# sangho-vision/acav100m

Measured on AMD Instinct MI355X. Metric: clips/sec curated (k-means train + assign, 2 views) + MI greedy selection of 20 %, higher is better.
Workload: dtype f32

## Files before the change

acav100m_amd/_lib.py:

```python
import ctypes as C
import os

_HERE = os.path.dirname(os.path.abspath(__file__))
LIB_PATH = os.environ.get("ACAV_LIB_PATH") or os.path.join(_HERE, "libacav_hip.so")

vp, i64, i32, f32, f64, u32 = C.c_void_p, C.c_int64, C.c_int, C.c_float, C.c_double, C.c_uint32
pp = C.POINTER(C.c_void_p)

SIGNATURES = {
    "acav_version": [],
    "acav_device_count": [C.POINTER(i32)],
    "acav_device_info": [i32, C.c_char_p, i32, C.POINTER(i32), C.POINTER(i64)],
    "acav_trim_device_cache": [C.POINTER(i64)],
    "acav_rng_create": [pp, u32],
    "acav_rng_destroy": [vp],
    "acav_rng_seed": [vp, u32],
    "acav_rng_u32": [vp, C.POINTER(u32)],
    "acav_rng_jump": [vp, i64],
    "acav_rng_py_shuffle": [vp, i64, vp],
    "acav_rng_rand_f32": [vp, vp, i64],
    "acav_rng_randperm": [vp, i64, vp],
    "acav_rng_get_state": [vp, vp, C.POINTER(i32)],
    "acav_rng_set_state": [vp, vp, i32],
    "acav_rng_warmup_best": [vp, i32, i64, vp, C.POINTER(f32)],
    "acav_kmeans_create": [pp, i32, i32, i32, vp, vp],
    "acav_kmeans_destroy": [vp],
    "acav_kmeans_get_state": [vp, vp, vp, C.POINTER(i64), C.POINTER(i64)],
    "acav_kmeans_set_state": [vp, vp, vp, i64, i64],
    "acav_kmeans_set_hyper": [vp, i32, f64, f64],
    "acav_kmeans_assign": [vp, vp, i64, vp, C.POINTER(f32)],
    "acav_kmeans_step": [vp, vp, i64, f64, vp, C.POINTER(f32)],
    "acav_kmeans_train": [vp, vp, i64, i64, f64, vp, i64],
    "acav_kmeans_train_multi": [vp, i32, vp, vp, i64, f64, vp, vp],
    "acav_kmeans_train_form": [i32, i32, i64, i32, i32, i32, i32, i32, i32, i32, C.POINTER(i32)],
    "acav_kmeans_assign_plan": [i32, i32, i64, i32, i32, i32, i32, C.POINTER(i32)],
    "acav_kmeans_apply_update": [vp, vp, i64, vp, f64],
    "acav_kmeans_sync": [vp],
    "acav_kmeans_shape": [vp, C.POINTER(i32), C.POINTER(i32)],
    "acav_kmeans_stream": [vp, pp],
    "acav_comm_unique_id": [vp],
    "acav_comm_init": [pp, i32, i32, i32, vp, vp],
    "acav_comm_destroy": [vp],
    "acav_comm_info": [vp, C.POINTER(i32), C.POINTER(i32)],
    "acav_comm_sync": [vp],
    "acav_comm_allreduce_f32": [vp, vp, i64],
    "acav_comm_allgather": [vp, vp, vp, i64],
    "acav_comm_broadcast": [vp, vp, i64, i32],
    "acav_kmeans_allreduce_init": [vp, vp],
    "acav_kmeans_train_dp": [vp, vp, vp, i64, i64, f64, vp, i64, i64, i32],
    "acav_kmeans_train_dp_multi": [vp, vp, i32, vp, i64, i64, f64, vp, vp, i64, vp],
    "acav_kmeans_train_plan_multi": [vp, vp, i32, vp, i64, i32, i64, vp, i64, i64, f64, vp, vp, i64, vp],
    "acav_kmeans_broadcast_state": [vp, vp, i32],
    "acav_kmeans_timer_begin": [vp],
    "acav_kmeans_timer_end": [vp, C.POINTER(f32)],
    "acav_kmeans_stats": [vp, C.POINTER(i64), C.POINTER(i64)],
    "acav_kmeans_train_stats": [vp, C.POINTER(i64), C.POINTER(i64)],
    "acav_kmeans_filter_stats": [vp, C.POINTER(i64), C.POINTER(i64), C.POINTER(i64)],
    "acav_kmeans_recheck_stats": [vp, C.POINTER(i64), C.POINTER(i64), C.POINTER(i64)],
    "acav_kmeans_filter_time": [vp, C.POINTER(f32)],
    "acav_contrastive_create": [pp, i32, i32, i32, i32, vp, vp],
    "acav_contrastive_destroy": [vp],
    "acav_contrastive_get_params": [vp, vp, C.POINTER(i64)],
    "acav_contrastive_set_params": [vp, vp],
    "acav_contrastive_train": [vp, vp, vp, vp, i64, f64, vp, vp],
    "acav_contrastive_infer": [vp, vp, vp, i64, vp],
    "acav_contrastive_set_comm": [vp, vp],
    "acav_contrastive_backward": [vp, vp, vp, i64, vp, vp],
    "acav_contrastive_get_grads": [vp, vp],
    "acav_contrastive_set_grads": [vp, vp],
    "acav_contrastive_step": [vp, f64],
    "acav_mi_create": [pp, i32, vp, i64, i32, i32, vp, i32, vp],
    "acav_mi_destroy": [vp],
    "acav_mi_add_samples": [vp, vp, i64],
    "acav_mi_score_batch": [vp, vp, i32, vp],
    "acav_mi_run_greedy": [vp, vp, i64, vp, i32, i64, i32, i32, i32, vp, vp, vp, C.POINTER(i64),
                           C.POINTER(i64), vp, vp, vp, vp, i64],
    "acav_mi_run_greedy_multi": [vp, i32, vp, vp, vp, vp, vp, i32, i32, i32, vp, vp, vp, vp, vp],
    "acav_fy_block_grid": [i32, i32, i32, C.POINTER(i64)],
    "acav_fy_block_map": [i64, i32, i32, i32, C.POINTER(i32), C.POINTER(i32), C.POINTER(i32)],
    "acav_mi_run_exact": [vp, vp, i64, i32, i64, vp, vp, C.POINTER(i64), vp, vp, vp],
    "acav_mi_run_exact_multi": [vp, i32, vp, vp, vp, vp, vp, vp, vp],
    "acav_mi_run_celf": [vp, vp, i64, i32, i64, f64, vp, vp, vp, C.POINTER(i64), i64, vp, vp, vp],
    "acav_mi_set_measure": [vp, i32],
    "acav_mi_set_average_method": [vp, i32],
    "acav_mi_set_pair_weights": [vp, vp, i32],
    "acav_mi_get_pair_stats": [vp, vp, vp, vp, vp],
    "acav_mi_get_counts": [vp, vp, vp, vp, C.POINTER(i64)],
    "acav_mi_sync": [vp],
    "acav_mi_timer_begin": [vp],
    "acav_mi_timer_end": [vp, C.POINTER(f32)],
    "acav_pkl_shard_open": [C.c_char_p, pp],
    "acav_pkl_shard_close": [vp],
    "acav_pkl_shard_info": [vp, C.POINTER(i64), C.POINTER(i32), C.POINTER(i32)],
    "acav_pkl_shard_view": [vp, i32, C.POINTER(i32), C.POINTER(C.c_char_p), C.POINTER(C.c_char_p), C.POINTER(C.c_char_p),
                            C.POINTER(C.c_char_p), C.POINTER(i64)],
    "acav_pkl_shard_copy_view": [vp, i32, vp, i64],
    "acav_pkl_shard_meta": [vp, pp, C.POINTER(i64), pp, C.POINTER(i64), pp, pp, pp],
    "acav_pkl_load_group": [vp, i32, vp, vp, i32, vp, vp, vp, vp, vp, i32, vp, vp],
    "acav_pkl_assign_load_group": [vp, i32, i32, vp, vp],
    "acav_pkl_shard_labels": [vp, pp],
}

_lib = None
_FIRST_DEVICE_CALLS = ("acav_device_count", "acav_device_info", "acav_kmeans_create", "acav_mi_create",
                       "acav_contrastive_create", "acav_comm_init")
_device_touched = False


def device_touched():
    return _device_touched


def _marking(fn):
    def call(*args):
        global _device_touched
        _device_touched = True
        return fn(*args)
    call.argtypes, call.restype, call.__name__ = fn.argtypes, fn.restype, fn.__name__
    return call


class AcavError(RuntimeError):
    pass


def load_library():
    global _lib
    if _lib is not None:
        return _lib
    if not os.path.exists(LIB_PATH):
        raise AcavError(
            f"{LIB_PATH} is missing: run `python __graft_entry__.py` (hipcc --offload-arch=gfx950) first. "
            "There is no CPU fallback.")
    try:
        import torch
    except Exception:
        pass
    lib = C.CDLL(LIB_PATH)
    lib.acav_last_error.restype = C.c_char_p
    lib.acav_last_error.argtypes = []
    for name, args in SIGNATURES.items():
        fn = getattr(lib, name)
        fn.restype = i32
        fn.argtypes = args
    for name in _FIRST_DEVICE_CALLS:
        setattr(lib, name, _marking(getattr(lib, name)))
    _lib = lib
    return lib


def check(rc):
    if rc != 0:
        msg = _lib.acav_last_error().decode("utf-8", "replace") if _lib is not None else ""
        if rc == -1:
            raise ValueError(f"acav: {msg}")
        if rc == -5:
            raise RuntimeError(f"acav: {msg}")
        if rc == -7:
            raise TimeoutError(f"acav: {msg}")
        raise AcavError(f"acav error {rc}: {msg}")


def device_count():
    n = i32(0)
    check(load_library().acav_device_count(C.byref(n)))
    return n.value


def ptr(obj):
    if obj is None:
        return None
    if hasattr(obj, "data_ptr"):
        return C.c_void_p(obj.data_ptr())
    return obj.ctypes.data_as(C.c_void_p)
```

acav100m_amd/csrc/acav_common.h:

```cpp
#pragma once
#include <hip/hip_runtime.h>

#include <cstdarg>
#include <cstdint>
#include <cstdio>
#include <cstring>
#include <new>
#include <vector>

#include "../../include/acav_hip.h"

#define ACAV_EXPORT extern "C" __attribute__((visibility("default")))

#if (defined(ACAV_ABL_NOAFRAG) || defined(ACAV_ABL_NOCDMA) || defined(ACAV_ABL_NOMFMA) || defined(ACAV_ABL_NOXDMA) || \
     defined(ACAV_ABL_NOXDMA_G123) || defined(ACAV_ABL_XHALF_G123) || \
     defined(ACAV_DBG_HALF_CAND_WINDOW) || defined(ACAV_FY_ABL_BKSEQ) || defined(ACAV_FY_ABL_NOWALK) || defined(ACAV_FY_ABL_SRCSEQ) || defined(ACAV_MI_ABL_EMPTY)) && \
    !defined(ACAV_EXPERIMENT_BUILD)
#error "ACAV_ABL_* / ACAV_FY_ABL_* / ACAV_MI_ABL_* select timing-only kernels with wrong results: experiment harnesses only (-DACAV_EXPERIMENT_BUILD)"
#endif

namespace acav {

void set_error(const char *fmt, ...);

#define ACAV_HIP_TRY(expr)                                                                         \
    do {                                                                                           \
        hipError_t _e = (expr);                                                                    \
        if (_e != hipSuccess) {                                                                    \
            acav::set_error("%s failed: %s (%s:%d)", #expr, hipGetErrorString(_e), __FILE__, __LINE__); \
            return ACAV_EHIP;                                                                      \
        }                                                                                          \
    } while (0)

#define ACAV_REQUIRE(cond, code, ...)      \
    do {                                   \
        if (!(cond)) {                     \
            acav::set_error(__VA_ARGS__);  \
            return (code);                 \
        }                                  \
    } while (0)

#define ACAV_TRY(expr)             \
    do {                           \
        int _rc = (expr);          \
        if (_rc != ACAV_OK) return _rc; \
    } while (0)

bool is_device_ptr(const void *p);

void retire_stream(hipStream_t s);
void retire_event(hipEvent_t e);
void flush_retired(bool force);
int devbuf_alloc(void **p, size_t *bytes, size_t want, int *dev = nullptr);
void devbuf_free(void *p, size_t bytes, int dev = -1);
size_t devbuf_trim();

struct DevBuf {
    void *p = nullptr;
    size_t bytes = 0;
    int dev = -1;
    hipStream_t owner = nullptr;
    bool bound = false;
    ~DevBuf() { release(); }
    void bind(hipStream_t s) { owner = s, bound = true; }
    void release()
    {
        if (p) devbuf_free(p, bytes, dev);
        p = nullptr;
        bytes = 0;
    }
    int ensure(size_t n)
    {
        if (n <= bytes) return ACAV_OK;
        if (p) (void)(bound ? hipStreamSynchronize(owner) : hipDeviceSynchronize());
        release();
        return devbuf_alloc(&p, &bytes, n, &dev);
    }
    template <class T> T *as() const { return static_cast<T *>(p); }
};

int to_device(const void *src, size_t bytes, DevBuf &stage, hipStream_t stream, const void **out);
int upload(DevBuf &dst, const void *src, size_t bytes, hipStream_t stream);
int from_device(void *dst, const void *src_dev, size_t bytes, hipStream_t stream);

const uint32_t *mt_jump_poly(int64_t J);
int mt_jump_window_host(uint32_t *window, int64_t J);

struct StreamCtx {
    int device = 0;
    hipStream_t stream = nullptr;
    bool own_stream = false;
    hipEvent_t ev0 = nullptr, ev1 = nullptr;
    int init(int dev, void *user_stream, int priority_class = 0);
    void fini(bool retire = false);
    int timer_begin();
    int timer_end(float *ms);
};

}
```

acav100m_amd/csrc/acav_mi.hip:

```cpp
#include <algorithm>
#include <chrono>
#include <cmath>
#include <type_traits>

#include "acav_common.h"
#include <rocprim/rocprim.hpp>
#include <vector>

using namespace acav;

#ifdef ACAV_MI_ABL_EMPTY
#define ACAV_MI_EMPTY_RETURN return;
#else
#define ACAV_MI_EMPTY_RETURN
#endif

namespace {

struct MiScalars {
    long long nc;
};

#ifdef ACAV_FY_PROF
__device__ unsigned long long fy_prof[16];
// ... 1159 lines not shown
    const bool before = r > 0 && celf_val_geq(pm[r - 1], qval[order[r]]);
    if (here && !before) dn->kstop = r + 1;
}
__global__ __launch_bounds__(256) void k_celf_dense_winner(int n, const double *__restrict__ d, const double *__restrict__ pm,
                                                           CelfDense *__restrict__ dn)
{
    const int r = blockIdx.x * 256 + threadIdx.x;
    const int k = dn->kstop;
    if (r >= k) return;
    const double best = pm[k - 1], v = d[r];
    if ((v != v && best != best) || v == best) atomicMax(&dn->winner, r);
}
__global__ __launch_bounds__(256) void k_celf_dense_apply(int n, const int *__restrict__ A, const int *__restrict__ order,
                                                          const double *__restrict__ d, const CelfDense *__restrict__ dn,
                                                          const CelfState *__restrict__ state, double *__restrict__ qval,
                                                          long long *__restrict__ qst, long long *__restrict__ tr_ids,
                                                          double *__restrict__ tr_vals, int tr_cap)
{
    const int r = blockIdx.x * 256 + threadIdx.x;
    if (r >= dn->kstop) return;
    const int w = order[r];
    qval[w] = d[r];
    qst[w] = state->t + r + 1;
    if (r < tr_cap) {
        if (tr_ids) tr_ids[r] = (long long)A[w];
        if (tr_vals) tr_vals[r] = d[r];
    }
}
template <bool PAIR>
__global__ __launch_bounds__(256) void k_celf_dense_commit(CelfCtx c, const int *__restrict__ A, const int *__restrict__ order,
                                                           const double *__restrict__ d, const CelfDense *__restrict__ dn,
                                                           CelfState *state, unsigned char *removed,
                                                           long long *__restrict__ S_out, double *__restrict__ G_out,
                                                           long long *__restrict__ LK_out, long long *__restrict__ tr_ids,
                                                           double *__restrict__ tr_vals, int tr_cap)
{
    const int tid = threadIdx.x;
    const int k = dn->kstop, a = dn->winner;
    const int pos = order[a];
    const long long nc = c.sc->nc;
    const double gain0 = state->gain;
    const long long t0 = state->t;
    __syncthreads();
    if (tid == 0) {
        long long lk = k;
        if (a != k - 1) {
            if (k < tr_cap) {
                if (tr_ids) tr_ids[k] = (long long)A[pos];
                if (tr_vals) tr_vals[k] = d[a];
            }
            ++lk;
        }
        removed[pos] = 1;
        state->gain = gain0 + d[a];
        state->t = t0 + lk;
        *S_out = (long long)A[pos];
        *G_out = gain0 + d[a];
        *LK_out = lk;
        c.sc->nc = nc + 1;
    }
    celf_commit_tables<PAIR>(c, A[pos], tid);
}

__global__ void k_celf_queue_out(int L, const unsigned char *__restrict__ removed, const double *__restrict__ qval,
                                 double *__restrict__ out)
{
    const int w = blockIdx.x * blockDim.x + threadIdx.x;
    if (w < L) out[w] = removed[w] ? -INFINITY : qval[w];
}

__device__ __forceinline__ unsigned mt_temper(unsigned y)
{
    y ^= y >> 11;
    y ^= (y << 7) & 0x9d2c5680u;
    y ^= (y << 15) & 0xefc60000u;
    y ^= y >> 18;
    return y;
}
__device__ __forceinline__ unsigned mt_twist(unsigned y) { return (y >> 1) ^ ((y & 1u) ? 0x9908b0dfu : 0u); }

constexpr int MT_THREADS = 640;
constexpr int MT_WIDE = 623;
constexpr int MT_BACK = 1078;
constexpr int MT_EPOCH = 24;
constexpr int MT_WIN = MT_BACK + MT_WIDE * MT_EPOCH;
__device__ __forceinline__ void mt_generate_body(const unsigned *__restrict__ mt_state, unsigned *__restrict__ out, long long n)
{
    __shared__ unsigned X[MT_WIN];
    const unsigned tid = threadIdx.x;
    if (n <= 0) return;
    const long long p = (long long)mt_state[624];
    for (unsigned k = tid; k < 624; k += MT_THREADS) X[k] = mt_state[k];
    const long long q = p + n;
    const long long need = 624 * ((q - 1) / 624) + 624;
    __syncthreads();
    for (long long m = p + tid; m < 624 && m < q; m += MT_THREADS) out[m - p] = X[m];
    unsigned *outp = out + (624 - p);
    long long m0 = 624;
    long long shift = 0;
    for (; m0 < need && m0 < MT_BACK; m0 += 227) {
        if (tid < 227) {
            const unsigned w = (unsigned)m0 + tid;
            const unsigned v = X[w - 227] ^ mt_twist((X[w - 624] & 0x80000000u) | (X[w - 623] & 0x7fffffffu));
            X[w] = v;
            if ((long long)w < q) outp[w - 624] = v;
        }
        asm volatile("s_waitcnt lgkmcnt(0)" ::: "memory");
        __builtin_amdgcn_s_barrier();
    }
    const unsigned *xw = X + ((unsigned)(m0 - shift) + tid - MT_BACK);
    unsigned ob = ((unsigned)(m0 - p) + tid) * 4u;
    const unsigned ob_end = (unsigned)n * 4u;
    const char *outb = reinterpret_cast<const char *>(out);
    int left = MT_EPOCH;
    while (m0 < need) {
        if (left == 0) {
            unsigned keep[2];
            const unsigned src = (unsigned)(m0 - shift) - MT_BACK;
#pragma unroll
            for (int u = 0; u < 2; ++u) keep[u] = tid + u * MT_THREADS < MT_BACK ? X[src + tid + u * MT_THREADS] : 0u;
#pragma unroll
            for (int u = 0; u < 2; ++u)
                if (tid + u * MT_THREADS < MT_BACK) X[tid + u * MT_THREADS] = keep[u];
            __syncthreads();
            shift = m0 - MT_BACK;
            xw = X + tid;
            left = MT_EPOCH;
        }
        if (tid < MT_WIDE) {
            const unsigned a = xw[0] ^ xw[227] ^ xw[454], b2 = xw[1] ^ xw[228] ^ xw[455];
            const unsigned v = xw[MT_BACK - 681] ^ mt_twist((a & 0x80000000u) | (b2 & 0x7fffffffu));
            const_cast<unsigned *>(xw)[MT_BACK] = v;
            if (ob < ob_end) *reinterpret_cast<unsigned *>(const_cast<char *>(outb) + ob) = v;
        }
        xw += MT_WIDE;
        ob += MT_WIDE * 4u;
        m0 += MT_WIDE;
        --left;
        asm volatile("s_waitcnt lgkmcnt(0)" ::: "memory");
        __builtin_amdgcn_s_barrier();
    }
    __syncthreads();
}

__global__ __launch_bounds__(MT_THREADS) void k_mt_generate_lanes(unsigned *__restrict__ states, unsigned *__restrict__ out0,
                                                                 long long blk, long long head)
{
    ACAV_MI_EMPTY_RETURN
    const long long lane = blockIdx.x;
    const long long extra = lane == 0 ? head : 0;
    mt_generate_body(states + lane * 625, out0 + lane * blk - extra, blk + extra);
}

constexpr int MJ_WORDS = MT_BACK + MT_WIDE * 32;
__global__ __launch_bounds__(MT_THREADS) void k_mt_jump(unsigned *__restrict__ states, int src0, int dst0,
                                                       const unsigned *__restrict__ poly)
{
    ACAV_MI_EMPTY_RETURN
    __shared__ unsigned X[MJ_WORDS];
    const unsigned tid = threadIdx.x;
    const unsigned *src = states + (size_t)(src0 + blockIdx.x) * 625;
    unsigned *dst = states + (size_t)(dst0 + blockIdx.x) * 625;
    for (unsigned k = tid; k < 624; k += MT_THREADS) X[k] = src[k];
    __syncthreads();
    for (unsigned m0 = 624; m0 < MT_BACK; m0 += 227) {
        if (tid < 227) {
            const unsigned w = m0 + tid;
            X[w] = X[w - 227] ^ mt_twist((X[w - 624] & 0x80000000u) | (X[w - 623] & 0x7fffffffu));
        }
        __syncthreads();
    }
    for (unsigned m0 = MT_BACK; m0 < MJ_WORDS; m0 += MT_WIDE) {
        if (tid < MT_WIDE) {
            const unsigned *xw = X + (m0 + tid - MT_BACK);
            const unsigned a = xw[0] ^ xw[227] ^ xw[454], b2 = xw[1] ^ xw[228] ^ xw[455];
            X[m0 + tid] = xw[MT_BACK - 681] ^ mt_twist((a & 0x80000000u) | (b2 & 0x7fffffffu));
        }
        __syncthreads();
    }
    if (tid < 624) {
        unsigned acc = 0u;
        const unsigned *xk = X + tid;
        for (int wi = 0; wi < 623; ++wi) {
            const unsigned g = poly[wi];
#pragma unroll
            for (int b = 0; b < 32; ++b) acc ^= xk[wi * 32 + b] & (0u - ((g >> b) & 1u));
        }
        acc ^= xk[623 * 32] & (0u - (poly[623] & 1u));
        dst[tid] = acc;
    }
    if (tid == 0) dst[624] = 624u;
}

__device__ __forceinline__ void fy_build_body(const unsigned *__restrict__ draws, int L, int *__restrict__ h,
                                              int *__restrict__ head, int *__restrict__ next, int *__restrict__ g, int i)
{
    if (i >= L) return;
    if (i == L - 1) {
        h[i] = i;
        next[i] = -1;
        return;
    }
    const int hh = i + (int)(mt_temper(draws[i]) % (unsigned)(L - i));
    h[i] = hh;
    if (hh != i) {
        next[i] = atomicExch(&head[hh], i);
        atomicMax(&g[hh], i);
    } else {
        next[i] = -1;
    }
}

__global__ __launch_bounds__(256) void k_fy_build(const unsigned *__restrict__ draws, int L, int *__restrict__ h,
                                                  int *__restrict__ head, int *__restrict__ next,
                                                  int *__restrict__ g)
{
    fy_build_body(draws, L, h, head, next, g, (int)(blockIdx.x * blockDim.x + threadIdx.x));
}

__device__ __forceinline__ void fy_apply_body(const int *__restrict__ A, int L, int B, const int *__restrict__ h,
                                              const int *__restrict__ head, const int *__restrict__ next,
                                              const int *__restrict__ g, int *__restrict__ batch_out,
                                              int *__restrict__ A_new, int *__restrict__ head_next,
                                              int *__restrict__ g_next, int i)
{
    if (i >= L) return;
    head_next[i] = -1;
    g_next[i] = -1;
    const int p = h[i];
    int j;
    if (p == i) {
        j = i;
    } else {
        int pred = -1;
        for (int q = head[p]; q >= 0; q = next[q])
            if (q < i && q > pred) pred = q;
        j = pred;
    }
    int src;
    if (j < 0) {
        src = p;
    } else {
        while (g[j] >= 0) j = g[j];
        src = j;
    }
    const int v = A[src];
    if (i < B)
        batch_out[i] = v;
    else
        A_new[i - B] = v;
}

__global__ __launch_bounds__(256) void k_fy_apply(const int *__restrict__ A, int L, int B,
                                                  const int *__restrict__ h, const int *__restrict__ head,
                                                  const int *__restrict__ next, const int *__restrict__ g,
                                                  int *__restrict__ batch_out, int *__restrict__ A_new,
                                                  int *__restrict__ head_next, int *__restrict__ g_next)
{
    fy_apply_body(A, L, B, h, head, next, g, batch_out, A_new, head_next, g_next, (int)(blockIdx.x * blockDim.x + threadIdx.x));
}

#ifndef ACAV_FYA_CH
#define ACAV_FYA_CH 8192
#endif
#ifndef ACAV_FYT_THREADS
#define ACAV_FYT_THREADS 1024
#endif
constexpr int FYA_CH = ACAV_FYA_CH;
constexpr int FYA_THREADS = 1024;
constexpr int64_t FY_TILED_MAX = 16 << 20;
constexpr unsigned FY_EREF = 0x80000000u;
// ... 463 lines not shown
    const int id = (int)threadIdx.x < B ? bprev[threadIdx.x] : 0;
    const bool feeds = it < c.iters && (int)threadIdx.x < nreq;
    const int dest = feeds ? c.tailinv[(size_t)(it % FY_NBUF) * SEL_MAXB + threadIdx.x] : 0;
    mi_select_body<W>(ss, c.asg, c.D, c.C, c.P, c.pairs, nullptr, id, bprev + SEL_MAXB, B, k, mode, c.Nc, c.ac, c.bc, c.SN, c.Sa, c.Sb,
                      c.phi, c.sc, nullptr, c.S + (size_t)ps * k, c.G + (size_t)ps * k, c.forced ? c.forced + (size_t)ps * k : nullptr,
                      c.tr_pos ? c.tr_pos + (size_t)ps * k : nullptr, c.tr_ids ? c.tr_ids + (size_t)ps * B : nullptr,
                      c.tr_sc ? c.tr_sc + (size_t)ps * B : nullptr, keep_unselected, sReq, 1, W ? c.w : nullptr);
    if (it >= c.iters || nreq == 0) return;
    lds_barrier();
    if (feeds) {
        const int v = sReq[threadIdx.x];
        if (dest < B) {
            int *bb = c.batch + (it & 1) * bstride;
            bb[dest] = v;
            for (int d = 0; d < c.D; ++d) bb[SEL_MAXB + dest * c.D + d] = c.asg[(size_t)v * c.D + d];
        } else {
            c.A[(it + 1) & 1][dest - B] = v;
        }
    }
}

__global__ void k_i64_to_i32(const long long *__restrict__ in, int *__restrict__ out, long long n)
{
    const long long i = (long long)blockIdx.x * blockDim.x + threadIdx.x;
    if (i < n) out[i] = (int)in[i];
}

}

struct acav_mi {
    StreamCtx ctx;
    int64_t V = 0;
    int D = 0, C = 0, P = 0;
    DevBuf asg, pairs, Nc, ac, bc, SN, Sa, Sb, phi, scalars;
    DevBuf stage, ids32, scores;
    DevBuf A0, A1, h, head, head2, next, g, g2, batch, S, G, tr_pos, tr_ids, tr_sc, forced;
    DevBuf removed, blockbest, ticket, tr_am;
    DevBuf celf_val, celf_stamp, celf_bv, celf_bst, celf_bp, celf_state, celf_lk, celf_qout;
    DevBuf celf_fresh, celf_ks, celf_ks2, celf_kv, celf_kv2, celf_i0, celf_i1, celf_i2, celf_d, celf_pm, celf_dn, celf_tmp;
    DevBuf chunk_desc;
    DevBuf chunk_blocks;
    DevBuf lane_states, ring, polys;
    DevBuf lnk, lf;
    int measure = 0;
    int avg = 0;
    DevBuf pst;
    bool weighted = false;
    bool pst_valid = false;
    int queue_probe_replaced = 0;
    bool lockstep_member = false;
    bool queue_probe_pending = false;
    bool prio_streams = false;
    int class_mt = 0, class_fy = 0;
    DevBuf fy_table, fy_bounds, fy_bucket, fy_count, fy_src[FY_GROUP], fy_g[FY_GROUP], fy_perm[FY_NBUF], fy_tail, fy_err;
    hipStream_t st_fy = nullptr;
    hipEvent_t ev_tile[FY_NBUF] = {}, ev_gather[FY_NBUF] = {};
    hipStream_t st_mt = nullptr;
    hipEvent_t ev_mt[2] = {nullptr, nullptr}, ev_used[2] = {nullptr, nullptr};
};

struct acav_rng;

static const float *mi_weights(acav_mi *mi)
{
    return mi->weighted ? reinterpret_cast<const float *>(mi->pairs.as<int>() + 2 * (size_t)mi->P) : nullptr;
}

static int mi_ensure_gen_events(acav_mi *mi);
struct MtStream {
    static constexpr int NSLOT = 2;
    static constexpr int64_t PAD = 624;
    static constexpr int64_t BLK_DEFAULT = 624 * 4096;
    int64_t T = 0, head = 0, blk = 0, S = 0, nblocks = 0, nsuper = 0, lmax = 0;
    int p0 = 0, W = 1, logW = 0;
    bool wraps = false;
    unsigned *ring = nullptr, *states = nullptr, *polys = nullptr;
    hipStream_t st = nullptr, smt = nullptr;
    hipEvent_t ev_mt[NSLOT] = {nullptr, nullptr}, ev_used[NSLOT] = {nullptr, nullptr};
    int64_t produced = 0;
    int64_t waited = -1;
    int64_t freed = 0;

    int plan(acav_mi *mi, hipStream_t consumer, const uint32_t *mtbuf, int idx, int64_t total_draws, int64_t L, int64_t span,
             hipStream_t generator = nullptr)
    {
        T = total_draws;
        p0 = idx;
        head = 624 - p0;
        lmax = L;
        const int64_t gen = T > head ? T - head : 0;
        if (gen <= BLK_DEFAULT) {
            W = 1;
            blk = 624 * ((gen + 623) / 624);
            nblocks = gen > 0 ? 1 : 0;
        } else {
            blk = BLK_DEFAULT;
            nblocks = (gen + blk - 1) / blk;
            W = 1;
            while (W < 32 && W < nblocks) W *= 2;
            if ((nblocks + W - 1) / W > NSLOT && (int64_t)W * blk < 2 * span) {
                blk = 624 * ((2 * span + 624 * (int64_t)W - 1) / (624 * (int64_t)W));
                nblocks = (gen + blk - 1) / blk;
            }
        }
        logW = 0;
        while ((1 << logW) < W) ++logW;
        S = (int64_t)W * blk;
        nsuper = nblocks ? (nblocks + W - 1) / W : 0;
        wraps = nsuper > NSLOT;
        st = consumer;
        smt = generator ? generator : mi->st_mt;
        ACAV_TRY(mi_ensure_gen_events(mi));
        for (int q = 0; q < NSLOT; ++q) ev_mt[q] = mi->ev_mt[q], ev_used[q] = mi->ev_used[q];
        const int64_t slots = nsuper < NSLOT ? nsuper : NSLOT;
        ACAV_TRY(mi->ring.ensure(sizeof(unsigned) * (size_t)(PAD + slots * S + (wraps ? lmax : 0) + 8)));
        ACAV_TRY(mi->lane_states.ensure(sizeof(unsigned) * 625 * (size_t)W));
        ring = mi->ring.as<unsigned>();
        states = mi->lane_states.as<unsigned>();
        uint32_t st0[625];
        memcpy(st0, mtbuf, 624 * sizeof(uint32_t));
        st0[624] = (uint32_t)p0;
        ACAV_HIP_TRY(hipMemcpyAsync(states, st0, sizeof(st0), hipMemcpyHostToDevice, st));
        if (head > 0) ACAV_HIP_TRY(hipMemcpyAsync(ring + PAD - head, mtbuf + p0, sizeof(unsigned) * (size_t)head, hipMemcpyHostToDevice, st));
        ACAV_HIP_TRY(hipStreamSynchronize(st));
        const int npoly = logW + 1;
        std::vector<uint32_t> hp((size_t)npoly * 624, 0u);
        for (int r = 0; r < npoly; ++r) {
            if (r == logW && nsuper <= 1) break;
            const uint32_t *g = mt_jump_poly(((int64_t)1 << r) * blk);
            ACAV_REQUIRE(g, ACAV_ESTATE, "could not derive the MT19937 jump polynomial");
            memcpy(&hp[(size_t)r * 624], g, 624 * sizeof(uint32_t));
        }
        ACAV_TRY(mi->polys.ensure(sizeof(uint32_t) * hp.size()));
        polys = mi->polys.as<unsigned>();
        ACAV_HIP_TRY(hipMemcpy(polys, hp.data(), sizeof(uint32_t) * hp.size(), hipMemcpyHostToDevice));
        produced = 0, waited = -1, freed = 0;
        ACAV_HIP_TRY(hipEventRecord(ev_used[0], st));
        ACAV_HIP_TRY(hipStreamWaitEvent(smt, ev_used[0], 0));
        for (int r = 0; r < logW; ++r)
            hipLaunchKernelGGL(k_mt_jump, dim3(1u << r), dim3(MT_THREADS), 0, smt, states, 0, 1 << r, polys + (size_t)r * 624);
        ACAV_HIP_TRY(hipGetLastError());
        for (int64_t q = 0; q < slots; ++q) ACAV_TRY(produce());
        return ACAV_OK;
    }
    int produce()
    {
        const int64_t s = produced++;
        const int slot = (int)(s % NSLOT);
        if (s >= NSLOT) ACAV_HIP_TRY(hipStreamWaitEvent(smt, ev_used[slot], 0));
        const int64_t left = nblocks - s * W;
        const unsigned lanes = (unsigned)(left < W ? left : W);
        unsigned *out0 = ring + PAD + (int64_t)slot * S;
        hipLaunchKernelGGL(k_mt_generate_lanes, dim3(lanes), dim3(MT_THREADS), 0, smt, states, out0, (long long)blk,
                           (long long)(s == 0 ? head : 0));
        if (s + 1 < nsuper)
            hipLaunchKernelGGL(k_mt_jump, dim3((unsigned)W), dim3(MT_THREADS), 0, smt, states, 0, 0, polys + (size_t)logW * 624);
        ACAV_HIP_TRY(hipGetLastError());
        if (wraps && slot == 0 && s > 0)
            ACAV_HIP_TRY(hipMemcpyAsync(ring + PAD + NSLOT * S, out0, sizeof(unsigned) * (size_t)lmax, hipMemcpyDeviceToDevice, smt));
        ACAV_HIP_TRY(hipEventRecord(ev_mt[slot], smt));
        return ACAV_OK;
    }
    int acquire(int64_t r0, int64_t n, const unsigned **ptr)
    {
        const int64_t r1 = r0 + n;
        const int64_t hi = r1 - 1 >= head ? (r1 - 1 - head) / S : -1;
        ACAV_REQUIRE(hi < produced, ACAV_ESTATE, "MT stream schedule: superblock %lld needed, %lld produced", (long long)hi,
                     (long long)produced);
        for (int64_t s = waited + 1; s <= hi; ++s) ACAV_HIP_TRY(hipStreamWaitEvent(st, ev_mt[s % NSLOT], 0));
        if (hi > waited) waited = hi;
        *ptr = r0 < head ? ring + PAD - head + r0 : ring + PAD + (r0 - head) % (NSLOT * S);
        return ACAV_OK;
    }
    int release(int64_t next_r0)
    {
        const int64_t lo = next_r0 >= head ? (next_r0 - head) / S : 0;
        while (freed < lo && freed < nsuper) {
            const int64_t s = freed++;
            if (s + NSLOT < nsuper) {
                ACAV_HIP_TRY(hipEventRecord(ev_used[s % NSLOT], st));
                ACAV_TRY(produce());
            }
        }
        return ACAV_OK;
    }
    int final_state(uint32_t *mtbuf, int *idx) const
    {
        const int64_t q = (int64_t)p0 + T;
        if (q <= 624) {
            *idx = (int)q;
            return ACAV_OK;
        }
        const int64_t base = 624 * ((q - 1) / 624);
        const int64_t r = base - p0;
        ACAV_HIP_TRY(hipMemcpy(mtbuf, ring + PAD + (r - head) % (NSLOT * S), 624 * sizeof(uint32_t), hipMemcpyDeviceToHost));
        *idx = (int)(q - base);
        return ACAV_OK;
    }
};

struct FyPlan {
    int gsh = 4, wcap = 256, ecap = 256, ecap_lds = 256, capg = 512, NT = 0;
    std::vector<unsigned short> table;
    std::vector<int> ebound;
    void build(int64_t L0)
    {
        int cap = 256, cap_max = 8192;
        if (const char *v = getenv("ACAV_FY_CAP")) {
            const int x = atoi(v);
            if (x >= 256 && x <= 8192 && (x & (x - 1)) == 0) cap_max = x;
        }
        int tiles_min = 32;
        if (const char *v = getenv("ACAV_FY_TILES_MIN")) tiles_min = atoi(v) > 0 ? atoi(v) : tiles_min;
        while (cap < cap_max && (int64_t)cap * tiles_min < L0) cap *= 2;
        wcap = ecap = cap;
        capg = (L0 + FYA_CH - 1) / FYA_CH >= 64 ? cap / 2 : 2 * cap;
        gsh = 0;
        while ((1 << gsh) < cap / 16) ++gsh;
        const int gran = 1 << gsh;
        const double limit = 0.7 * ecap, lnL = log((double)L0);
        table.assign((size_t)((L0 + gran - 1) >> gsh) + 1, 0);
        ebound.clear();
        int64_t e = 0;
        while (e < L0) {
            int width = 0;
            double mass = 0.0;
            do {
                const double x = (double)(e + width);
                const double m = gran * (lnL - log(x + 1.0)) + 1.0;
                if (width > 0 && mass + (m > 0 ? m : 0) > limit) break;
                mass += m > 0 ? m : 0;
                width += gran;
            } while (width < wcap && e + width < L0);
            const int t = (int)ebound.size();
            ebound.push_back((int)e);
// ... 504 lines not shown
    }
    ACAV_HIP_TRY(hipStreamSynchronize(st));
    for (int c = 0; c < nchunks; ++c) {
        ACAV_HIP_TRY(hipStreamSynchronize(streams[(size_t)c].smt ? streams[(size_t)c].smt : mis[c]->st_mt));
        unsigned mtbuf[625];
        int idx = 0;
        ACAV_TRY(acav_rng_get_state(rngs[c], mtbuf, &idx));
        ACAV_TRY(streams[(size_t)c].final_state(mtbuf, &idx));
        ACAV_TRY(acav_rng_set_state(rngs[c], mtbuf, idx));
        unsigned ferr = 0;
        ACAV_HIP_TRY(hipMemcpy(&ferr, mis[c]->fy_err.p, sizeof(ferr), hipMemcpyDeviceToHost));
        ACAV_REQUIRE(ferr == 0, ACAV_ESTATE, "tiled Fisher-Yates: a tile bucket of chunk %d overflowed (flags %u); re-run with "
                                             "ACAV_FY_LEGACY=1", c, ferr);
    }
    if (timing)
        fprintf(stderr, "[acav]   set-up %.1f ms (per-chunk work %.1f: add_samples %.1f, ids %.1f, tables %.1f, generator plan %.1f; then the sync), "
                        "read-back + generator states %.1f ms\n", t_setup, t_chunks, t_add, t_ids, t_fy, t_mt, ms_since(t_tail0));
    return ACAV_OK;
}

ACAV_EXPORT int acav_fy_block_grid(int nx, int ny, int gz, int64_t *blocks)
{
    ACAV_REQUIRE(blocks, ACAV_EINVAL, "NULL argument");
    ACAV_REQUIRE(nx > 0 && ny > 0 && gz > 0 && (int64_t)ny * gz < (1 << 24), ACAV_EINVAL, "bad grid %d x %d x %d", nx, ny, gz);
    *blocks = fy_affine_blocks((unsigned)nx, (unsigned)ny, (unsigned)gz);
    return ACAV_OK;
}

ACAV_EXPORT int acav_fy_block_map(int64_t b, int nx, int ny, int gz, int *x, int *y, int *z)
{
    ACAV_REQUIRE(x && y && z, ACAV_EINVAL, "NULL argument");
    ACAV_REQUIRE(nx > 0 && ny > 0 && gz > 0 && (int64_t)ny * gz < (1 << 24), ACAV_EINVAL, "bad grid %d x %d x %d", nx, ny, gz);
    const long long nb = fy_affine_blocks((unsigned)nx, (unsigned)ny, (unsigned)gz);
    ACAV_REQUIRE(nb <= 0x7fffffffll && b >= 0 && b < nb, ACAV_EINVAL, "workgroup %lld outside the grid of %lld", (long long)b, nb);
    const FyBlock q = fy_block_map((unsigned)b, (unsigned)nx, (unsigned)ny, (unsigned)gz);
    *x = q.work ? q.x : -1, *y = q.work ? q.y : -1, *z = q.work ? q.z : -1;
    return ACAV_OK;
}

ACAV_EXPORT int acav_mi_run_greedy_multi(acav_mi **mis, int nchunks, const int64_t *const *candidates, const int64_t *L,
                                         const int64_t *const *start, const int *ns, const int64_t *subset, int B, int k,
                                         int keep_unselected, acav_rng **rngs, int64_t *const *S_out,
                                         double *const *GAIN_out, int64_t *n_selected, int64_t *n_iters)
{
    ACAV_REQUIRE(mis && nchunks > 0 && candidates && L && ns && subset && rngs && S_out && GAIN_out, ACAV_EINVAL,
                 "NULL argument");
    ACAV_REQUIRE(B > 0 && B <= SEL_WIDEB && k > 0 && k <= B, ACAV_EINVAL,
                 "batch_size %d / selection_size %d out of range (1 <= selection_size <= batch_size <= %d)", B, k, SEL_WIDEB);
    acav_mi *lead = mis[0];
    ACAV_REQUIRE(lead, ACAV_EINVAL, "handle is NULL");
    for (int c = 0; c < nchunks; ++c)
        if (mis[c]) mis[c]->pst_valid = false;
    ACAV_HIP_TRY(hipSetDevice(lead->ctx.device));
    const char *legacy = getenv("ACAV_FY_LEGACY");
    bool tiled = !(legacy && legacy[0] == '1');
    for (int c = 0; c < nchunks; ++c) {
        acav_mi *mi = mis[c];
        ACAV_TRY(check_chunk_args(c, mi, candidates[c], L[c], start ? start[c] : nullptr, ns[c], subset[c], rngs[c], S_out[c], GAIN_out[c]));
        ACAV_REQUIRE(mi->ctx.device == lead->ctx.device, ACAV_EINVAL, "chunk %d lives on another device", c);
        ACAV_REQUIRE((int64_t)B * mi->P <= SEL_MAXBP, ACAV_EINVAL, "chunk %d: batch_size %d x %d pairs exceeds B*P <= %d", c, B, mi->P,
                     SEL_MAXBP);
        for (int e = 0; e < c; ++e)
            ACAV_REQUIRE(mis[e] != mi && rngs[e] != rngs[c], ACAV_EINVAL, "chunks must not share a handle or a generator");
        tiled = tiled && L[c] <= FY_TILED_MAX;
    }
    if (tiled)
        return run_greedy_tiled(mis, nchunks, candidates, L, start, ns, subset, B, k, keep_unselected, rngs, S_out, GAIN_out,
                                n_selected, n_iters, TiledExtras());
    const int64_t dl = B - (keep_unselected ? B - k : 0);
    for (int c = 0; c < nchunks; ++c) {
        const GreedyPlan gp = greedy_plan(L[c], subset[c], B, k, dl, -1);
        ACAV_REQUIRE(gp.short_l < 0, ACAV_ERANGE, "chunk %d: %lld candidates left < batch_size %d (batch.py:143-150)", c,
                     (long long)gp.short_l, B);
    }
    for (int c = 0; c < nchunks; ++c) {
        ACAV_HIP_TRY(hipStreamSynchronize(mis[c]->ctx.stream));
        ACAV_TRY(run_greedy_legacy(mis[c], candidates[c], L[c], start ? start[c] : nullptr, ns[c], subset[c], B, k, keep_unselected,
                                   rngs[c], S_out[c], GAIN_out[c], n_selected ? n_selected + c : nullptr,
                                   n_iters ? n_iters + c : nullptr, TiledExtras()));
    }
    return ACAV_OK;
}

ACAV_EXPORT int acav_mi_set_measure(acav_mi *mi, int measure)
{
    ACAV_REQUIRE(mi, ACAV_EINVAL, "handle is NULL");
    ACAV_REQUIRE(measure >= 0 && measure <= 6, ACAV_EINVAL, "unknown measure %d", measure);
    ACAV_REQUIRE(measure != 2 || (int64_t)mi->C <= mi->V + 1, ACAV_EINVAL, "nmi: ncentroids %d exceeds the ln k table (V + 1 = %lld)",
                 mi->C, (long long)(mi->V + 1));
    if ((measure == 1 || measure == 2) && !mi->lnk.p) {
        ACAV_HIP_TRY(hipSetDevice(mi->ctx.device));
        std::vector<double> lnk((size_t)mi->V + 2), lf((size_t)mi->V + 2);
        lnk[0] = 0.0, lf[0] = 0.0;
        for (int64_t k = 1; k < mi->V + 2; ++k) lnk[(size_t)k] = log((double)k), lf[(size_t)k] = lgamma((double)k + 1.0);
        ACAV_TRY(mi->lnk.ensure(sizeof(double) * lnk.size()));
        ACAV_TRY(mi->lf.ensure(sizeof(double) * lf.size()));
        ACAV_HIP_TRY(hipMemcpyAsync(mi->lnk.p, lnk.data(), sizeof(double) * lnk.size(), hipMemcpyHostToDevice, mi->ctx.stream));
        ACAV_HIP_TRY(hipMemcpyAsync(mi->lf.p, lf.data(), sizeof(double) * lf.size(), hipMemcpyHostToDevice, mi->ctx.stream));
        ACAV_HIP_TRY(hipStreamSynchronize(mi->ctx.stream));
    }
    mi->measure = measure;
    return ACAV_OK;
}

ACAV_EXPORT int acav_mi_set_average_method(acav_mi *mi, int method)
{
    ACAV_REQUIRE(mi, ACAV_EINVAL, "handle is NULL");
    ACAV_REQUIRE(method >= 0 && method <= 2, ACAV_EINVAL, "unknown average_method %d (0 arithmetic, 1 max, 2 min)", method);
    mi->avg = method;
    return ACAV_OK;
}

ACAV_EXPORT int acav_mi_set_pair_weights(acav_mi *mi, const float *weights, int P)
{
    ACAV_REQUIRE(mi, ACAV_EINVAL, "handle is NULL");
    if (!weights) {
        mi->weighted = false;
        return ACAV_OK;
    }
    ACAV_REQUIRE(P == mi->P, ACAV_EINVAL, "%d pair weights for a handle of %d pairs", P, mi->P);
    ACAV_REQUIRE(!is_device_ptr(weights), ACAV_EINVAL, "weights are a host array");
    for (int p = 0; p < P; ++p)
        ACAV_REQUIRE(std::isfinite(weights[p]), ACAV_EINVAL, "pair weight %d is not finite", p);
    ACAV_HIP_TRY(hipSetDevice(mi->ctx.device));
    ACAV_HIP_TRY(hipMemcpyAsync(mi->pairs.as<int>() + 2 * (size_t)P, weights, sizeof(float) * (size_t)P, hipMemcpyHostToDevice,
                                mi->ctx.stream));
    ACAV_HIP_TRY(hipStreamSynchronize(mi->ctx.stream));
    mi->weighted = true;
    return ACAV_OK;
}

static int pair_stats_init(acav_mi *mi, hipStream_t on = nullptr)
{
    if (mi->pst_valid) return ACAV_OK;
    ACAV_TRY(mi->pst.ensure(sizeof(PairStat) * (size_t)mi->P));
    hipLaunchKernelGGL(k_pair_stats_init, dim3(mi->P), dim3(256), 0, on ? on : mi->ctx.stream, mi->C, mi->Nc.as<int>(), mi->ac.as<int>(),
                       mi->bc.as<int>(), mi->pst.as<PairStat>());
    ACAV_HIP_TRY(hipGetLastError());
    mi->pst_valid = true;
    return ACAV_OK;
}

ACAV_EXPORT int acav_mi_get_pair_stats(acav_mi *mi, int64_t *TP, int64_t *FP, int64_t *FN, int64_t *TN)
{
    ACAV_REQUIRE(mi, ACAV_EINVAL, "handle is NULL");
    ACAV_HIP_TRY(hipSetDevice(mi->ctx.device));
    hipStream_t st = mi->ctx.stream;
    ACAV_TRY(pair_stats_init(mi));
    std::vector<PairStat> ps((size_t)mi->P);
    ACAV_HIP_TRY(hipMemcpyAsync(ps.data(), mi->pst.p, sizeof(PairStat) * ps.size(), hipMemcpyDeviceToHost, st));
    MiScalars s{};
    ACAV_HIP_TRY(hipMemcpyAsync(&s, mi->scalars.p, sizeof(s), hipMemcpyDeviceToHost, st));
    ACAV_HIP_TRY(hipStreamSynchronize(st));
    const long long n2 = s.nc * (s.nc - 1) / 2;
    for (int p = 0; p < mi->P; ++p) {
        const PairStat &q = ps[(size_t)p];
        if (TP) TP[p] = q.tab;
        if (FP) FP[p] = q.ta - q.tab;
        if (FN) FN[p] = q.tb - q.tab;
        if (TN) TN[p] = ((n2 - q.ta) - q.tb) + q.tab;
    }
    return ACAV_OK;
}

ACAV_EXPORT int acav_mi_run_exact(acav_mi *mi, const int64_t *candidates, int64_t L, int ns, int64_t subset,
                                  int64_t *S_out, double *GAIN_out, int64_t *n_selected, const int64_t *forced_pos,
// ... 579 lines not shown
```

include/acav_hip.h:

```cpp
#ifndef ACAV_HIP_H
#define ACAV_HIP_H

#include <stddef.h>
#include <stdint.h>

#ifdef __cplusplus
extern "C" {
#endif

#define ACAV_OK 0
#define ACAV_EINVAL (-1)
#define ACAV_EHIP (-2)
#define ACAV_ENOMEM (-3)
#define ACAV_ESTATE (-4)
#define ACAV_ERANGE (-5)
#define ACAV_EUNSUPPORTED (-6)
#define ACAV_ETIMEOUT (-7)

typedef struct acav_rng acav_rng;
typedef struct acav_kmeans acav_kmeans;
typedef struct acav_mi acav_mi;

const char *acav_last_error(void);
int acav_version(void);
// ... 1 lines not shown
int acav_device_info(int device, char *name, int name_len, int *compute_units, int64_t *hbm_bytes);
int acav_trim_device_cache(int64_t *freed_bytes);

int acav_rng_create(acav_rng **out, uint32_t seed);
int acav_rng_destroy(acav_rng *rng);
int acav_rng_seed(acav_rng *rng, uint32_t seed);
int acav_rng_u32(acav_rng *rng, uint32_t *out);
int acav_rng_jump(acav_rng *rng, int64_t n);
int acav_rng_py_shuffle(acav_rng *rng, int64_t n, int64_t *out_host);
int acav_rng_rand_f32(acav_rng *rng, float *out_host, int64_t n);
int acav_rng_randperm(acav_rng *rng, int64_t n, int64_t *out_host);
int acav_rng_get_state(const acav_rng *rng, uint32_t *mt624, int *idx);
int acav_rng_set_state(acav_rng *rng, const uint32_t *mt624, int idx);
int acav_rng_warmup_best(acav_rng *rng, int k, int64_t b, int64_t *best_host, float *mean_out);

int acav_kmeans_create(acav_kmeans **out, int device, int k, int d, const float *centers0, void *stream);
int acav_kmeans_destroy(acav_kmeans *km);
int acav_kmeans_get_state(acav_kmeans *km, float *centers, float *counts, int64_t *count, int64_t *fallback);
int acav_kmeans_set_state(acav_kmeans *km, const float *centers, const float *counts, int64_t count,
                          int64_t fallback);
int acav_kmeans_set_hyper(acav_kmeans *km, int initial_rounds, double reinit_p, double reinit_r);
int acav_kmeans_assign(acav_kmeans *km, const float *x, int64_t n, int64_t *labels, float *mean_dist);
int acav_kmeans_step(acav_kmeans *km, const float *x, int64_t b, double lr, const int64_t *forced_best,
                     float *mean_dist);
int acav_kmeans_train(acav_kmeans *km, const float *x, int64_t n, int64_t b, double lr,
                      const int64_t *warm_best, int64_t n_warm);
int acav_kmeans_train_multi(acav_kmeans *const *kms, int count, const float *const *xs, const int64_t *ns, int64_t b,
                            double lr, const int64_t *const *warm_best, const int64_t *n_warm);
int acav_kmeans_train_form(int d, int k, int64_t b, int aligned, int cus, int occ_narrow, int occ_split, int has_budget,
                           int room, int share_lds, int *out);
#define ACAV_ASSIGN_PLAN_LEN 27
int acav_kmeans_assign_plan(int d, int k, int64_t n, int aligned, int need_mean, int rows_scaled, int cus, int *out);
int acav_kmeans_apply_update(acav_kmeans *km, const float *x, int64_t b, const int64_t *best, double lr);
int acav_kmeans_sync(acav_kmeans *km);
int acav_kmeans_shape(const acav_kmeans *km, int *k, int *d);
int acav_kmeans_stream(const acav_kmeans *km, void **stream);
int acav_kmeans_timer_begin(acav_kmeans *km);
int acav_kmeans_timer_end(acav_kmeans *km, float *ms);
int acav_kmeans_filter_stats(acav_kmeans *km, int64_t *filter_launches, int64_t *rows, int64_t *rechecked);
int acav_kmeans_recheck_stats(acav_kmeans *km, int64_t *cand_rows, int64_t *cand_pairs, int64_t *full_rows);
int acav_kmeans_filter_time(acav_kmeans *km, float *ms);
int acav_kmeans_stats(acav_kmeans *km, int64_t *assign_launches, int64_t *step_launches);
int acav_kmeans_train_stats(acav_kmeans *km, int64_t *persistent_launches, int64_t *persistent_fallbacks);

typedef struct acav_comm acav_comm;
int acav_comm_unique_id(uint8_t *id128);
int acav_comm_init(acav_comm **out, int device, int rank, int world, const uint8_t *id128, void *stream);
int acav_comm_destroy(acav_comm *comm);
int acav_comm_info(const acav_comm *comm, int *rank, int *world);
int acav_comm_sync(acav_comm *comm);
int acav_comm_allreduce_f32(acav_comm *comm, float *buf_dev, int64_t n);
int acav_comm_allgather(acav_comm *comm, const void *send_dev, void *recv_dev, int64_t bytes);
int acav_comm_broadcast(acav_comm *comm, void *buf_dev, int64_t bytes, int root);
int acav_kmeans_allreduce_init(acav_kmeans *km, acav_comm *comm);
int acav_kmeans_train_dp(acav_kmeans *km, acav_comm *comm, const float *x_local_dev, int64_t n_local, int64_t b_local,
                         double lr, const int64_t *warm_global, int64_t n_warm, int64_t chunk_steps, int flags);
#define ACAV_DP_TRAIN 1
#define ACAV_DP_NOWAIT 2
#define ACAV_DP_ROOTED 4
int acav_kmeans_train_dp_multi(acav_kmeans *const *kms, acav_comm *const *comms, int count, const float *const *x_local_dev,
                               int64_t n_local, int64_t b_local, double lr, const int64_t *const *warm_global,
                               const int64_t *n_warm, int64_t chunk_steps, const int *train_here);
int acav_kmeans_train_plan_multi(acav_kmeans *const *kms, acav_comm *const *comms, int count, const float *const *x_local_dev,
                                 int64_t n_local, int slots, int64_t lb, const int64_t *ext, int64_t n_ext, int64_t steps,
                                 double lr, const int64_t *const *warm_global, const int64_t *n_warm, int64_t chunk_steps,
                                 const int *train_here);
int acav_kmeans_broadcast_state(acav_kmeans *km, acav_comm *comm, int root);

int acav_mi_create(acav_mi **out, int device, const int64_t *assignments, int64_t V, int D, int C,
                   const int32_t *pairs, int P, void *stream);
int acav_mi_destroy(acav_mi *mi);
int acav_mi_add_samples(acav_mi *mi, const int64_t *ids, int64_t n);
int acav_mi_score_batch(acav_mi *mi, const int64_t *ids, int B, double *scores_host);
int acav_mi_run_greedy(acav_mi *mi, const int64_t *candidates, int64_t L, const int64_t *start, int ns,
                       int64_t subset, int B, int k, int keep_unselected, acav_rng *rng, int64_t *S_out,
                       double *GAIN_out, int64_t *n_selected, int64_t *n_iters, int64_t *trace_ids,
                       double *trace_scores, int32_t *trace_pos, const int32_t *forced_pos, int64_t max_iters);
int acav_mi_run_greedy_multi(acav_mi **mis, int nchunks, const int64_t *const *candidates, const int64_t *L,
                             const int64_t *const *start, const int *ns, const int64_t *subset, int B, int k,
                             int keep_unselected, acav_rng **rngs, int64_t *const *S_out, double *const *GAIN_out,
                             int64_t *n_selected, int64_t *n_iters);
int acav_fy_block_grid(int nx, int ny, int gz, int64_t *blocks);
int acav_fy_block_map(int64_t b, int nx, int ny, int gz, int *x, int *y, int *z);
int acav_mi_set_measure(acav_mi *mi, int measure);
int acav_mi_set_average_method(acav_mi *mi, int method);
int acav_mi_set_pair_weights(acav_mi *mi, const float *weights, int P);
int acav_mi_get_pair_stats(acav_mi *mi, int64_t *TP, int64_t *FP, int64_t *FN, int64_t *TN);
int acav_mi_run_exact(acav_mi *mi, const int64_t *candidates, int64_t L, int ns, int64_t subset, int64_t *S_out,
                      double *GAIN_out, int64_t *n_selected, const int64_t *forced_pos, double *trace_scores,
                      int64_t *trace_argmax);
int acav_mi_run_exact_multi(acav_mi **mis, int nchunks, const int64_t *const *candidates, const int64_t *L,
                            const int *ns, const int64_t *subset, int64_t *const *S_out, double *const *GAIN_out,
                            int64_t *n_selected);
int acav_mi_run_celf(acav_mi *mi, const int64_t *candidates, int64_t L, int ns, int64_t subset, double celf_ratio,
                     int64_t *S_out, double *GAIN_out, int64_t *LOOKUPS_out, int64_t *n_selected, int64_t trace_cap,
                     int64_t *trace_ids, double *trace_vals, double *queue_final);
int acav_mi_get_counts(acav_mi *mi, int32_t *N, int32_t *a, int32_t *b, int64_t *n);
int acav_mi_sync(acav_mi *mi);
int acav_mi_timer_begin(acav_mi *mi);
int acav_mi_timer_end(acav_mi *mi, float *ms);

typedef struct acav_contrastive acav_contrastive;
int acav_contrastive_create(acav_contrastive **out, int device, int visual_size, int audio_size, int out_size,
                            const float *params_host, void *stream);
int acav_contrastive_destroy(acav_contrastive *c);
int acav_contrastive_get_params(acav_contrastive *c, float *params_host, int64_t *step);
int acav_contrastive_set_params(acav_contrastive *c, const float *params_host);
int acav_contrastive_train(acav_contrastive *c, const float *visual, const float *audio, const int64_t *offsets,
                           int64_t nbatches, double lr, float *losses, float *accs);
int acav_contrastive_infer(acav_contrastive *c, const float *visual, const float *audio, int64_t n, float *logits_host);
int acav_contrastive_set_comm(acav_contrastive *c, acav_comm *comm);
int acav_contrastive_backward(acav_contrastive *c, const float *visual, const float *audio, int64_t n, float *loss, float *acc);
int acav_contrastive_get_grads(acav_contrastive *c, float *grads_host);
int acav_contrastive_set_grads(acav_contrastive *c, const float *grads_host);
int acav_contrastive_step(acav_contrastive *c, double lr);

typedef struct acav_pkl_shard acav_pkl_shard;
int acav_pkl_shard_open(const char *path, acav_pkl_shard **out);
int acav_pkl_shard_close(acav_pkl_shard *s);
int acav_pkl_shard_info(const acav_pkl_shard *s, int64_t *rows, int *nviews, int *n_names);
int acav_pkl_shard_view(const acav_pkl_shard *s, int v, int *kind, const char **model_key, const char **layer,
                        const char **extractor, const char **dataset, int64_t *d);
int acav_pkl_shard_copy_view(const acav_pkl_shard *s, int v, float *dst, int64_t row_stride);
int acav_pkl_shard_meta(const acav_pkl_shard *s, const char **filenames, int64_t *filenames_len, const char **names,
                        int64_t *names_len, const int64_t **name_ids, const int64_t **name_of_row,
                        const int64_t **shard_size);
int acav_pkl_load_group(const char *const *paths, int n, const int64_t *base, const int64_t *n_expect, int nviews,
                        const int *kinds, const char *const *model_keys, const char *const *layers, const int64_t *dims,
                        float *const *dest, int threads, acav_pkl_shard **handles, int *status);
int acav_pkl_assign_load_group(const char *const *paths, int n, int threads, acav_pkl_shard **handles, int *status);
int acav_pkl_shard_labels(const acav_pkl_shard *s, const int64_t **labels);

#ifdef __cplusplus
}
#endif
#endif
```

Measured before the change: 592,000.

## Shrink Mersenne Twister LDS window so generator co-resides with FY tile kernel

```diff
diff --git a/acav100m_amd/_lib.py b/acav100m_amd/_lib.py
--- a/acav100m_amd/_lib.py
+++ b/acav100m_amd/_lib.py
@@ -86,6 +86,7 @@
     "acav_mi_set_pair_weights": [vp, vp, i32],
     "acav_mi_get_pair_stats": [vp, vp, vp, vp, vp],
     "acav_mi_get_counts": [vp, vp, vp, vp, C.POINTER(i64)],
+    "acav_mt_stream_fill": [vp, i32, i64, i64, i32, vp],
     "acav_mi_sync": [vp],
     "acav_mi_timer_begin": [vp],
     "acav_mi_timer_end": [vp, C.POINTER(f32)],
@@ -103,7 +104,7 @@
 
 _lib = None
 _FIRST_DEVICE_CALLS = ("acav_device_count", "acav_device_info", "acav_kmeans_create", "acav_mi_create",
-                       "acav_contrastive_create", "acav_comm_init")
+                       "acav_contrastive_create", "acav_comm_init", "acav_mt_stream_fill")
 _device_touched = False
 
 
diff --git a/acav100m_amd/csrc/acav_common.h b/acav100m_amd/csrc/acav_common.h
--- a/acav100m_amd/csrc/acav_common.h
+++ b/acav100m_amd/csrc/acav_common.h
@@ -14,9 +14,10 @@
 
 #if (defined(ACAV_ABL_NOAFRAG) || defined(ACAV_ABL_NOCDMA) || defined(ACAV_ABL_NOMFMA) || defined(ACAV_ABL_NOXDMA) || \
      defined(ACAV_ABL_NOXDMA_G123) || defined(ACAV_ABL_XHALF_G123) || \
-     defined(ACAV_DBG_HALF_CAND_WINDOW) || defined(ACAV_FY_ABL_BKSEQ) || defined(ACAV_FY_ABL_NOWALK) || defined(ACAV_FY_ABL_SRCSEQ) || defined(ACAV_MI_ABL_EMPTY)) && \
+     defined(ACAV_DBG_HALF_CAND_WINDOW) || defined(ACAV_FY_ABL_BKSEQ) || defined(ACAV_FY_ABL_NOWALK) || defined(ACAV_FY_ABL_SRCSEQ) || defined(ACAV_MI_ABL_EMPTY) || \
+     defined(ACAV_MT_ABL_STALE)) && \
     !defined(ACAV_EXPERIMENT_BUILD)
-#error "ACAV_ABL_* / ACAV_FY_ABL_* / ACAV_MI_ABL_* select timing-only kernels with wrong results: experiment harnesses only (-DACAV_EXPERIMENT_BUILD)"
+#error "ACAV_ABL_* / ACAV_FY_ABL_* / ACAV_MI_ABL_* / ACAV_MT_ABL_* select timing-only kernels with wrong results: experiment harnesses only (-DACAV_EXPERIMENT_BUILD)"
 #endif
 
 namespace acav {
diff --git a/acav100m_amd/csrc/acav_mi.hip b/acav100m_amd/csrc/acav_mi.hip
--- a/acav100m_amd/csrc/acav_mi.hip
+++ b/acav100m_amd/csrc/acav_mi.hip
@@ -1265,8 +1265,18 @@
 constexpr int MT_THREADS = 640;
 constexpr int MT_WIDE = 623;
 constexpr int MT_BACK = 1078;
-constexpr int MT_EPOCH = 24;
+#ifndef ACAV_MT_EPOCH
+#define ACAV_MT_EPOCH 9
+#define ACAV_MT_EPOCH_DEFAULT
+#endif
+constexpr int MT_EPOCH = ACAV_MT_EPOCH;
 constexpr int MT_WIN = MT_BACK + MT_WIDE * MT_EPOCH;
+constexpr size_t lds_granules(size_t bytes) { return (bytes + 1279) / 1280 * 1280; }
+static_assert(MT_EPOCH >= 2, "the slide moves the last MT_BACK words to the front: the two ranges must be disjoint");
+#ifdef ACAV_MT_EPOCH_DEFAULT
+static_assert(lds_granules(sizeof(unsigned) * MT_WIN) + lds_granules(8192 * 16 + 1024 ) <= 160 * 1024,
+              "a generator workgroup and a k_fy_tile_multi workgroup at the largest tile must fit on one CU together");
+#endif
 __device__ __forceinline__ void mt_generate_body(const unsigned *__restrict__ mt_state, unsigned *__restrict__ out, long long n)
 {
     __shared__ unsigned X[MT_WIN];
@@ -1335,12 +1345,12 @@
     mt_generate_body(states + lane * 625, out0 + lane * blk - extra, blk + extra);
 }
 
-constexpr int MJ_WORDS = MT_BACK + MT_WIDE * 32;
+constexpr unsigned MJ_NEED = 624 + 19937 - 1;
 __global__ __launch_bounds__(MT_THREADS) void k_mt_jump(unsigned *__restrict__ states, int src0, int dst0,
                                                        const unsigned *__restrict__ poly)
 {
     ACAV_MI_EMPTY_RETURN
-    __shared__ unsigned X[MJ_WORDS];
+    __shared__ unsigned X[MT_WIN];
     const unsigned tid = threadIdx.x;
     const unsigned *src = states + (size_t)(src0 + blockIdx.x) * 625;
     unsigned *dst = states + (size_t)(dst0 + blockIdx.x) * 625;
@@ -1353,23 +1363,50 @@
         }
         __syncthreads();
     }
-    for (unsigned m0 = MT_BACK; m0 < MJ_WORDS; m0 += MT_WIDE) {
-        if (tid < MT_WIDE) {
-            const unsigned *xw = X + (m0 + tid - MT_BACK);
-            const unsigned a = xw[0] ^ xw[227] ^ xw[454], b2 = xw[1] ^ xw[228] ^ xw[455];
-            X[m0 + tid] = xw[MT_BACK - 681] ^ mt_twist((a & 0x80000000u) | (b2 & 0x7fffffffu));
-        }
+    unsigned m0 = MT_BACK;
+    unsigned shift = 0;
+    unsigned wdone = 0;
+    unsigned acc = 0u;
+    for (;;) {
+        for (int e = 0; e < MT_EPOCH && m0 < MJ_NEED; ++e, m0 += MT_WIDE) {
+            if (tid < MT_WIDE) {
+                unsigned *xw = X + (m0 - shift + tid - MT_BACK);
+                const unsigned a = xw[0] ^ xw[227] ^ xw[454], b2 = xw[1] ^ xw[228] ^ xw[455];
+                xw[MT_BACK] = xw[MT_BACK - 681] ^ mt_twist((a & 0x80000000u) | (b2 & 0x7fffffffu));
+            }
+            __syncthreads();
+        }
+        const unsigned wfull = (m0 - 623u) >> 5, wend = wfull < 623u ? wfull : 623u;
+        if (tid < 624) {
+            auto poly_at = [&](unsigned w) { return poly[w < 624u ? w : 623u]; };
+            unsigned pnext = poly_at(wdone + (tid & 31u));
+            for (unsigned w0 = wdone; w0 < wend; w0 += 32u) {
+                const unsigned pv = pnext;
+                pnext = poly_at(w0 + 32u + (tid & 31u));
+                const unsigned cnt = wend - w0 < 32u ? wend - w0 : 32u;
+                for (unsigned j = 0; j < cnt; ++j) {
+                    const unsigned g = __builtin_amdgcn_readlane(pv, j);
+                    const unsigned *xk = X + ((w0 + j) * 32u - shift + tid);
+#pragma unroll
+                    for (int b = 0; b < 32; ++b) acc ^= xk[b] & (0u - ((g >> b) & 1u));
+                }
+            }
+        }
+        wdone = wend;
+        if (m0 >= MJ_NEED) break;
         __syncthreads();
+        unsigned keep[2];
+        const unsigned from = m0 - shift - MT_BACK;
+#pragma unroll
+        for (int u = 0; u < 2; ++u) keep[u] = tid + u * MT_THREADS < MT_BACK ? X[from + tid + u * MT_THREADS] : 0u;
+#pragma unroll
+        for (int u = 0; u < 2; ++u)
+            if (tid + u * MT_THREADS < MT_BACK) X[tid + u * MT_THREADS] = keep[u];
+        __syncthreads();
+        shift = m0 - MT_BACK;
     }
     if (tid < 624) {
-        unsigned acc = 0u;
-        const unsigned *xk = X + tid;
-        for (int wi = 0; wi < 623; ++wi) {
-            const unsigned g = poly[wi];
-#pragma unroll
-            for (int b = 0; b < 32; ++b) acc ^= xk[wi * 32 + b] & (0u - ((g >> b) & 1u));
-        }
-        acc ^= xk[623 * 32] & (0u - (poly[623] & 1u));
+        acc ^= X[623u * 32u - shift + tid] & (0u - (poly[623] & 1u));
         dst[tid] = acc;
     }
     if (tid == 0) dst[624] = 624u;
@@ -1999,14 +2036,18 @@
     int64_t freed = 0;
 
     int plan(acav_mi *mi, hipStream_t consumer, const uint32_t *mtbuf, int idx, int64_t total_draws, int64_t L, int64_t span,
-             hipStream_t generator = nullptr)
+             hipStream_t generator = nullptr, int64_t force_blk = 0, int force_W = 0)
     {
         T = total_draws;
         p0 = idx;
         head = 624 - p0;
         lmax = L;
         const int64_t gen = T > head ? T - head : 0;
-        if (gen <= BLK_DEFAULT) {
+        if (force_blk > 0) {
+            blk = force_blk;
+            nblocks = (gen + blk - 1) / blk;
+            W = force_W;
+        } else if (gen <= BLK_DEFAULT) {
             W = 1;
             blk = 624 * ((gen + 623) / 624);
             nblocks = gen > 0 ? 1 : 0;
@@ -2068,6 +2109,12 @@
         const int64_t left = nblocks - s * W;
         const unsigned lanes = (unsigned)(left < W ? left : W);
         unsigned *out0 = ring + PAD + (int64_t)slot * S;
+#ifdef ACAV_MT_ABL_STALE
+        if (s >= NSLOT) {
+            ACAV_HIP_TRY(hipEventRecord(ev_mt[slot], smt));
+            return ACAV_OK;
+        }
+#endif
         hipLaunchKernelGGL(k_mt_generate_lanes, dim3(lanes), dim3(MT_THREADS), 0, smt, states, out0, (long long)blk,
                            (long long)(s == 0 ? head : 0));
         if (s + 1 < nsuper)
@@ -2738,6 +2785,41 @@
     return ACAV_OK;
 }
 
+ACAV_EXPORT int acav_mt_stream_fill(const uint32_t *state, int idx, int64_t n_words, int64_t blk, int W, uint32_t *out)
+{
+    ACAV_REQUIRE(state && out && idx >= 0 && idx <= 624 && n_words > 0 && n_words < ((int64_t)1 << 40), ACAV_EINVAL, "bad argument");
+    ACAV_REQUIRE(blk >= 624 && blk % 624 == 0 && blk < ((int64_t)1 << 29) - 624, ACAV_EINVAL, "blk: a multiple of 624 below 2^29 - 624");
+    ACAV_REQUIRE(W >= 1 && W <= 32 && (W & (W - 1)) == 0, ACAV_EINVAL, "W: a power of two up to 32");
+    ACAV_REQUIRE(!is_device_ptr(out), ACAV_EINVAL, "out is a host array");
+    acav_mi *mi = new (std::nothrow) acav_mi;
+    ACAV_REQUIRE(mi, ACAV_ENOMEM, "out of host memory");
+    int rc = mi->ctx.init(0, nullptr);
+    if (rc != ACAV_OK) {
+        delete mi;
+        return rc;
+    }
+    auto body = [&]() -> int {
+        ACAV_TRY(mi_ensure_streams(mi));
+        hipStream_t st = mi->ctx.stream;
+        const int64_t span = (int64_t)W * blk / 2;
+        MtStream ms;
+        ACAV_TRY(ms.plan(mi, st, state, idx, n_words, span, span, nullptr, blk, W));
+        for (int64_t r0 = 0; r0 < n_words; r0 += span) {
+            const int64_t n = n_words - r0 < span ? n_words - r0 : span;
+            const unsigned *draws = nullptr;
+            ACAV_TRY(ms.acquire(r0, n, &draws));
+            ACAV_HIP_TRY(hipMemcpyAsync(out + r0, draws, sizeof(uint32_t) * (size_t)n, hipMemcpyDeviceToHost, st));
+            ACAV_TRY(ms.release(r0 + n));
+        }
+        ACAV_HIP_TRY(hipStreamSynchronize(st));
+        ACAV_HIP_TRY(hipStreamSynchronize(mi->st_mt));
+        return ACAV_OK;
+    };
+    rc = body();
+    const int rc2 = acav_mi_destroy(mi);
+    return rc != ACAV_OK ? rc : rc2;
+}
+
 ACAV_EXPORT int acav_mi_set_measure(acav_mi *mi, int measure)
 {
     ACAV_REQUIRE(mi, ACAV_EINVAL, "handle is NULL");
diff --git a/include/acav_hip.h b/include/acav_hip.h
--- a/include/acav_hip.h
+++ b/include/acav_hip.h
@@ -107,6 +107,7 @@
                              int64_t *n_selected, int64_t *n_iters);
 int acav_fy_block_grid(int nx, int ny, int gz, int64_t *blocks);
 int acav_fy_block_map(int64_t b, int nx, int ny, int gz, int *x, int *y, int *z);
+int acav_mt_stream_fill(const uint32_t *state, int idx, int64_t n_words, int64_t blk, int W, uint32_t *out);
 int acav_mi_set_measure(acav_mi *mi, int measure);
 int acav_mi_set_average_method(acav_mi *mi, int method);
 int acav_mi_set_pair_weights(acav_mi *mi, const float *weights, int P);
```

Measured after the change: 598,000, median of 6. 1.01x the previous value.
